# mitenjain/nanopore

Hardware: AMD Instinct MI355X
Metric: DP cells/sec (banded pair-HMM realign: forward + backward + posterior per cell) (higher is better)
Workload: dtype f32

## Files before the change

### nanopore_amd/csrc/npr_api_internal.h

```cpp
#pragma once
#include <hip/hip_runtime.h>

#include <algorithm>
#include <atomic>
#include <chrono>
#include <cmath>
#include <cstdio>
#include <cstdlib>
#include <cstring>
#include <exception>
#include <memory>
#include <mutex>
#include <new>
#include <numeric>
#include <string>
#include <thread>
#include <type_traits>
#include <vector>

#include "npr_device.h"
#include "npr_internal.h"
#include "npr_sched.h"
#include "npr_threads.h"

using namespace npr;

struct npr_plan {
    Plan plan;
};

namespace npr_impl {
struct MeaScratch;

struct DeviceArena {
    static constexpr size_t kPad = 1024;
    std::mutex mu;
    char *F = nullptr;
    std::atomic<size_t> cells{0};
    std::atomic<uint64_t> epoch{1};
    int users = 0;
};
constexpr int kMaxDevices = 64;
extern DeviceArena g_arena[kMaxDevices];
}
using namespace npr_impl;

struct npr_ctx {
    int device = -1;
    hipStream_t stream = nullptr;
    hipEvent_t ev0 = nullptr, ev1 = nullptr;
    static constexpr int kSideStreams = 6;
    hipStream_t side[kSideStreams] = {};
    hipEvent_t side_done[kSideStreams] = {};
    int cu_count = 0;
    size_t total_mem = 0;
    bool model_set[NPR_MAX_MODELS] = {};
    DevModel models[NPR_MAX_MODELS];
    DevModel *d_models = nullptr;
    std::string last_error;
    int host_threads = 1;
    DeviceArena *arena = nullptr;
    int overlap = 0;
    int64_t opt[NPR_OPT_COUNT] = {};
    static constexpr size_t kArenaPad = DeviceArena::kPad;
    float *arena_Fx = nullptr;
    size_t arena_fx_cells = 0;
    void *pin_pairs = nullptr;
    size_t pin_pairs_bytes = 0;
    std::vector<hipEvent_t> ops_events;
    struct HostWords {
        std::unique_ptr<uint32_t[]> p;
        int64_t cap = 0;
    };
    std::vector<HostWords> packed_pool;
    void take_packed(int64_t words, std::unique_ptr<uint32_t[]> &p, int64_t &cap) {
        for (size_t i = 0; i < packed_pool.size(); ++i)
            if (packed_pool[i].cap >= words) {
                p = std::move(packed_pool[i].p), cap = packed_pool[i].cap;
                packed_pool.erase(packed_pool.begin() + static_cast<std::ptrdiff_t>(i));
                return;
            }
    }
    void give_packed(std::unique_ptr<uint32_t[]> &p, int64_t cap) {
        if (!p) return;
        if (packed_pool.size() < 2) {
            packed_pool.push_back(HostWords{std::move(p), cap});
            return;
        }
        auto &smallest = *std::min_element(packed_pool.begin(), packed_pool.end(), [](const HostWords &x, const HostWords &y) { return x.cap < y.cap; });
        if (smallest.cap < cap) smallest.p = std::move(p), smallest.cap = cap;
    }
    void *pin_stage = nullptr;
    size_t pin_stage_bytes = 0;
    MeaScratch *mea = nullptr;
    struct Cached {
        void *p;
        size_t bytes;
    };
    std::vector<Cached> cache;
    size_t cache_bytes = 0;
    void cache_flush() {
        for (const Cached &c : cache) (void)hipFree(c.p);
        cache.clear();
        cache_bytes = 0;
// ... 113 lines not shown
struct StageTimer {
    bool on;
    std::chrono::steady_clock::time_point t0;
    const char *what;
    explicit StageTimer(const char *w) : on(std::getenv("NPR_TIMING") != nullptr), t0(std::chrono::steady_clock::now()), what(w) {}
    void lap(const char *label) {
        if (!on) return;
        const auto t1 = std::chrono::steady_clock::now();
        std::fprintf(stderr, "[npr timing] %s / %s: %.1f ms\n", what, label, std::chrono::duration<double, std::milli>(t1 - t0).count());
        t0 = t1;
    }
};

}
using namespace npr_impl;

struct npr_batch {
    npr_ctx *ctx = nullptr;
    npr_params params{};
    int64_t n_reads = 0;
    std::vector<int64_t> ref_len, read_len;
    std::vector<int64_t> gstart;
    std::vector<int32_t> ref_id;
    std::vector<int32_t> guide_ops;
    std::vector<int64_t> guide_off;
    std::vector<int32_t> read_status;
    std::vector<int32_t> read_first_task, read_ntasks;
    std::vector<Task> tasks;
    std::vector<int32_t> task_of;
    std::vector<int64_t> task_cells;
    std::vector<TaskOut> outs;
    std::vector<uint8_t> task_rerun;
    npr_batch_stats stats{};
    DevBuf<Task> d_tasks;
    DevBuf<TaskOut> d_outs;
    DevBuf<int32_t> d_queue;
    DevBuf<uint8_t> d_seq;
    DevBuf<int32_t> d_lo, d_n;
    DevBuf<uint32_t> d_coff;
    DevBuf<uint32_t> d_ctl;
    DevBuf<Stripe> d_stripes;
    DevBuf<uint32_t> d_rowmask;
    DevBuf<PlanSeg> d_pseg;
    DevBuf<int64_t> d_region;
    std::vector<int64_t> region_end;
    size_t scratch_cells = 0;
    bool variable_regions = false;
    bool pair_rs = false;
    DevBuf<int32_t> d_px, d_py;
    DevBuf<float> d_pp;
    int64_t slot_stride = 0;
    struct Launch {
        int cls;
        int first, count, grid, wcap;
        int threads;
        size_t lds;
        int64_t cells;
        int64_t width;
        int slot_base;
        int region_first;
        bool own_regions;
    };
    std::vector<Launch> launches;
    DevBuf<float> d_ring;
    bool ran = false, finished = false;
    int32_t finish_stage = 0;
    std::vector<npr_read_result> results;
    std::vector<int64_t> ops_off;
    std::unique_ptr<int32_t[]> ops;
    int64_t ops_words = 0, ops_cap = 0;
    std::unique_ptr<uint32_t[]> packed;
    int64_t packed_cap = 0;
    bool have_pairs_form = false, have_packed_form = false;
    bool ops_from_guide = false;
    bool rs_staged = false;
    int rs_shift = 0;
    std::vector<int64_t> rs_columns, rs_kept;
    DevBuf<int32_t> d_rs_gy;
    DevBuf<int64_t> d_rs_gx_off;
    std::vector<int64_t> pair_off;
    std::vector<Pair> pairs;
    bool pairs_ready = false;
    std::vector<int64_t> task_dst;
    const uint32_t *dev_ops = nullptr;
    const int64_t *dev_od = nullptr;
    uint64_t dev_ops_epoch = 0;
    std::unique_ptr<char[]> text;
    int64_t text_cap = 0;
    std::vector<int64_t> text_off;
    bool text_ready = false, words_on_device = false;
};

struct npr_pileup {
    npr_ctx *ctx = nullptr;
    std::vector<int64_t> len;
    std::vector<int64_t> base;
    int64_t rows = 0;
    DevBuf<int32_t> tab;
    DevBuf<int32_t> diff;
    DevBuf<int32_t> tile;
    DevBuf<int64_t> dbase;
    DevBuf<int32_t> bad;
};

namespace npr_impl {

inline bool build_stair_schedule(const Segment &s, int R, int NW, uint32_t *ctl, int64_t *cells) {
    if (s.n.empty()) return false;
    return stair_schedule(s.lo.data(), s.n.data(), s.D(), s.max_width, R, NW, ctl, cells);
}

}
using namespace npr_impl;

namespace npr_impl {
enum { K_STAIR = 0, K_WIDE = 1, K_GENERIC_LDS = 2, K_GENERIC_GLOBAL = 3, K_TILE = 4, K_MID = 5, K_RS = 6, K_TILE_RS = 7 };
struct KClass {
    int kind, R, NW;
    int slots() const { return 64 * R * NW; }
};
constexpr int kClasses = 19;
constexpr KClass kClassTab[kClasses] = {{K_STAIR, 1, 1}, {K_STAIR, 2, 1}, {K_STAIR, 4, 1}, {K_WIDE, 2, 4}, {K_WIDE, 2, 8},
                                        {K_WIDE, 4, 8}, {K_WIDE, 4, 12}, {K_GENERIC_LDS, 0, 0}, {K_GENERIC_LDS, 0, 0},
                                        {K_GENERIC_LDS, 0, 0}, {K_GENERIC_GLOBAL, 0, 0}, {K_TILE, 2, 0},
                                        {K_MID, 1, 1}, {K_MID, 2, 1}, {K_MID, 4, 1},
                                        {K_RS, 1, 1}, {K_RS, 2, 1}, {K_RS, 4, 1},
                                        {K_TILE_RS, 2, 0}};
constexpr int kFirstGeneric = 7, kTileClass = 11, kFirstPair = 12, kFirstRs = 15, kTileRsClass = 18, kQueueSlots = 24;
inline bool is_register_class(int c) { return kClassTab[c].kind <= K_WIDE || kClassTab[c].kind == K_MID || kClassTab[c].kind == K_RS; }
inline bool is_one_wave_kind(int kind) { return kind == K_STAIR || kind == K_RS; }
inline bool is_tile_kind(int kind) { return kind == K_TILE || kind == K_TILE_RS; }
inline int stair_waves_per_cu(int R) { return R == 1 ? 28 : (R == 2 ? 24 : 12); }
inline int rs_waves_per_cu(int R) { return R == 1 ? 28 : (R == 2 ? 28 : 16); }

inline bool rs_model_ok(const DevModel &m) {
    double grow = 0.0, em_max = 0.0;
    for (int x = 0; x < 4; ++x)
        for (int y = 0; y < 4; ++y) em_max = std::max(em_max, static_cast<double>(m.em[x * 5 + y]));
    for (int to = 0; to < 5; ++to) {
        double col = 0.0, e = em_max;
        for (int from = 0; from < 5; ++from) col += static_cast<double>(m.T[from * 5 + to]);
        if (to > 0) {
            e = 0.0;
            for (int b2 = 0; b2 < 5; ++b2) e = std::max(e, static_cast<double>((to == 1 || to == 3) ? m.ex[to * 5 + b2] : m.ey[to * 5 + b2]));
        }
        grow = std::max(grow, col * e);
    }
    auto emax = [&](int st) {
        if (st == 0) return em_max;
        double e = 0.0;
        for (int b2 = 0; b2 < 5; ++b2) e = std::max(e, static_cast<double>((st == 1 || st == 3) ? m.ex[st * 5 + b2] : m.ey[st * 5 + b2]));
        return e;
    };
    for (int from = 0; from < 5; ++from) {
        double row = 0.0;
        for (int to = 0; to < 5; ++to) row += static_cast<double>(m.T[from * 5 + to]) * emax(to);
        grow = std::max(grow, row);
    }
    return grow <= std::exp2(6.0 / NPR_RS_K);
}

struct ModelShape { bool sw, flat_gaps, flat, rs_ok; };
inline ModelShape model_shape(const npr_ctx *ctx) {
    ModelShape s{false, true, false, true};
    for (int sl = 0; sl < NPR_MAX_MODELS; ++sl) {
        if (!ctx->model_set[sl]) continue;
        const DevModel &m = ctx->models[sl];
        if (m.T[1 * 5 + 2] != 0.f || m.T[2 * 5 + 1] != 0.f) s.sw = true;
        if (!rs_model_ok(m)) s.rs_ok = false;
        for (int b2 = 0; b2 < 5; ++b2)
            if (m.ex[5 + b2] != 0.25f || m.ex[15 + b2] != 0.25f || m.ey[10 + b2] != 0.25f || m.ey[20 + b2] != 0.25f) s.flat_gaps = false;
    }
    s.flat = !s.sw && s.flat_gaps;
    return s;
}

inline void build_stripes(const Segment &s, int R, Stripe *out, int64_t *rows_out) {
    const int64_t S = (s.xe - s.xs) / (64 * R) + 1;
    int64_t rows;
    if (out) {
        rows = stripe_ranges(s.lo.data(), s.n.data(), s.D(), s.xe - s.xs, R, &out[1].df, &out[1].dl, static_cast<int>(sizeof(Stripe) / sizeof(int32_t)));
        stripe_fill(out, s.xe - s.xs, R);
    } else {
        thread_local std::vector<int32_t> df, dl;
        df.resize(S), dl.resize(S);
        rows = stripe_ranges(s.lo.data(), s.n.data(), s.D(), s.xe - s.xs, R, df.data(), dl.data(), 1);
    }
    if (rows_out) *rows_out = rows;
}
inline int64_t stripes_of(const Segment &s, int R) { return (s.xe - s.xs) / (64 * R) + 1; }
}
using namespace npr_impl;

namespace npr_impl {
int32_t rescore_stage(npr_batch *b);
KernelArgs make_args(npr_batch *b);
int32_t ensure_coff(npr_batch *b);
int32_t release_scratch(npr_ctx *ctx, bool caches_only);
void ensure_packed_form(npr_batch *b);
int32_t grow_pin_stage(npr_ctx *ctx, size_t bytes, const char *what);
int32_t device_words_text(npr_batch *b, const int64_t *d_off, const uint32_t *d_words, char *lend, size_t lend_bytes);
using PieceMove = void (*)(void *dst, const void *pin, int64_t lo, int64_t hi);
struct PiecedFetch {
    const void *dev;
    void *dst;
    int64_t count;
    size_t elem;
    int64_t per_piece, round_to;
    PieceMove move;
    const char *what_pin, *what_d2h;
};
int32_t fetch_pieced(npr_ctx *ctx, const PiecedFetch &f);
int32_t fetch_device_words(npr_batch *b);
}
```

### nanopore_amd/csrc/npr_finish.cpp

```cpp
#include "npr_api_internal.h"

namespace npr_impl {

static int32_t grow_pinned(npr_ctx *ctx, void *&p, size_t &have, size_t bytes, const char *what) {
    if (bytes <= have) return NPR_OK;
    if (p) (void)hipHostFree(p);
    p = nullptr, have = 0;
    const hipError_t e = hipHostMalloc(&p, bytes + bytes / 4, hipHostMallocDefault);
    if (e != hipSuccess) return fail(ctx, NPR_ERR_NOMEM, what, e);
    have = bytes + bytes / 4;
    return NPR_OK;
}
int32_t grow_pin_pairs(npr_ctx *ctx, size_t bytes, const char *what) { return grow_pinned(ctx, ctx->pin_pairs, ctx->pin_pairs_bytes, bytes, what); }
int32_t grow_pin_stage(npr_ctx *ctx, size_t bytes, const char *what) { return grow_pinned(ctx, ctx->pin_stage, ctx->pin_stage_bytes, bytes, what); }

int32_t fetch_pieced(npr_ctx *ctx, const PiecedFetch &f) {
    if (f.count <= 0) return NPR_OK;
    const int32_t grown = grow_pin_pairs(ctx, f.elem * static_cast<size_t>(f.count), f.what_pin);
    if (grown != NPR_OK) return grown;
    constexpr int64_t kMaxPieces = 48;
    const int64_t pieces = std::min(kMaxPieces, (f.count + f.per_piece - 1) / f.per_piece);
    const int64_t piece = ((f.count + pieces - 1) / pieces + f.round_to - 1) / f.round_to * f.round_to;
    while (static_cast<int64_t>(ctx->ops_events.size()) < pieces) {
        hipEvent_t ev;
// ... 112 lines not shown
        int64_t runs = 0, cols = 0, kept = 0;
        for (int64_t q = b->guide_off[i]; q < b->guide_off[i + 1]; ++q) {
            const int32_t len = b->guide_ops[2 * q + 1];
            kept += len > 0;
            if (b->guide_ops[2 * q] == NPR_OP_M && len > 0) ++runs, cols += len;
        }
        b->rs_columns[i] = cols, b->rs_kept[i] = kept, run_off[i + 1] = b->read_status[i] == NPR_OK ? runs : 0;
    });
    if (ctx->opt[NPR_OPT_HOST_MEA] != 0 || n == 0) return NPR_OK;
    int e2 = 0;
    (void)std::frexp(b->params.posterior_threshold, &e2);
    const int shift = 24 - e2;
    if (!(b->params.posterior_threshold > 0.0) || shift > 44 || shift < 0) return NPR_OK;
    for (int64_t i = 0; i < n; ++i) {
        if (b->rs_columns[i] >= (int64_t(1) << (53 - shift))) return NPR_OK;
        run_off[i + 1] += run_off[i];
        gx_off[i + 1] = gx_off[i] + (b->read_status[i] == NPR_OK ? b->ref_len[i] + 1 : 0);
    }
    std::vector<int32_t> runs_v;
    int32_t *runs = nullptr;
    const size_t run_bytes = sizeof(int32_t) * 3 * static_cast<size_t>(run_off[n]);
    if (ctx->pin_stage && ctx->pin_stage_bytes >= run_bytes) runs = static_cast<int32_t *>(ctx->pin_stage);
    else runs_v.resize(3 * static_cast<size_t>(run_off[n])), runs = runs_v.data();
    parallel_for(n, ctx->host_threads, [&](int64_t i) {
        if (b->read_status[i] != NPR_OK) return;
        int32_t *out = runs + 3 * run_off[i];
        int64_t x = 0, y = 0;
        for (int64_t q = b->guide_off[i]; q < b->guide_off[i + 1]; ++q) {
            const int32_t op = b->guide_ops[2 * q], len = b->guide_ops[2 * q + 1];
            if (op == NPR_OP_M) {
                if (len > 0) out[0] = static_cast<int32_t>(x), out[1] = static_cast<int32_t>(y), out[2] = len, out += 3;
                x += len, y += len;
            } else if (op == NPR_OP_I) {
                y += len;
            } else {
                x += len;
            }
        }
    });
    tm.lap("runs");
    DevBuf<int64_t> d_run_off;
    DevBuf<int32_t> d_runs;
    hipError_t e;
    if ((e = d_run_off.alloc_from(ctx, n + 1)) != hipSuccess || (e = b->d_rs_gx_off.alloc_from(ctx, n + 1)) != hipSuccess ||
        (e = d_runs.alloc_from(ctx, std::max<size_t>(3 * static_cast<size_t>(run_off[n]), 1))) != hipSuccess ||
        (e = b->d_rs_gy.alloc_from(ctx, std::max<int64_t>(gx_off[n], 1))) != hipSuccess)
        return fail(ctx, NPR_ERR_NOMEM, "npr_batch_create: hipMalloc (rescore tables)", e);
    HIP_TRY(ctx, hipMemcpyAsync(d_run_off.p, run_off.data(), sizeof(int64_t) * (n + 1), hipMemcpyHostToDevice, ctx->stream));
    HIP_TRY(ctx, hipMemcpyAsync(b->d_rs_gx_off.p, gx_off.data(), sizeof(int64_t) * (n + 1), hipMemcpyHostToDevice, ctx->stream));
    if (run_bytes) HIP_TRY(ctx, hipMemcpyAsync(d_runs.p, runs, run_bytes, hipMemcpyHostToDevice, ctx->stream));
    HIP_TRY(ctx, hipMemsetAsync(b->d_rs_gy.p, 0xff, sizeof(int32_t) * std::max<int64_t>(gx_off[n], 1), ctx->stream));
    RescoreArgs ra{static_cast<int32_t>(n), 0, d_run_off.p, d_runs.p, b->d_rs_gx_off.p, b->d_rs_gy.p, nullptr, nullptr, nullptr, nullptr, nullptr, nullptr, shift};
    const int rc = launch_rescore_table(ra, ctx->stream);
    if (rc != 0) return fail(ctx, NPR_ERR_HIP, "k_rescore_table launch", static_cast<hipError_t>(rc));
    HIP_TRY(ctx, hipStreamSynchronize(ctx->stream));
    tm.lap("table");
    b->rs_shift = shift, b->rs_staged = true;
    return NPR_OK;
}

int32_t rescore_sum(npr_batch *b, std::vector<double> &score) {
    npr_ctx *ctx = b->ctx;
    const int64_t n = b->n_reads, ntasks = static_cast<int64_t>(b->tasks.size());
    DevBuf<unsigned long long> d_sum;
    hipError_t e;
    if ((e = d_sum.alloc_from(ctx, n)) != hipSuccess) return fail(ctx, NPR_ERR_NOMEM, "npr_batch_finish: hipMalloc (rescore sums)", e);
    HIP_TRY(ctx, hipMemsetAsync(d_sum.p, 0, sizeof(unsigned long long) * n, ctx->stream));
    RescoreArgs ra{static_cast<int32_t>(n), static_cast<int32_t>(ntasks), nullptr, nullptr, b->d_rs_gx_off.p, b->d_rs_gy.p, b->d_tasks.p, b->d_outs.p,
                   b->d_px.p, b->d_py.p, b->d_pp.p, d_sum.p, b->rs_shift};
    const int rc = launch_rescore_sum(ra, ctx->stream);
    if (rc != 0) return fail(ctx, NPR_ERR_HIP, "k_rescore_sum launch", static_cast<hipError_t>(rc));
    std::vector<unsigned long long> sum(n);
    HIP_TRY(ctx, hipMemcpyAsync(sum.data(), d_sum.p, sizeof(unsigned long long) * n, hipMemcpyDeviceToHost, ctx->stream));
    HIP_TRY(ctx, hipStreamSynchronize(ctx->stream));
    score.assign(n, 0.0);
    for (int64_t i = 0; i < n; ++i)
        if (b->rs_columns[i] > 0) score[i] = std::ldexp(static_cast<double>(sum[i]), -b->rs_shift) / static_cast<double>(b->rs_columns[i]);
    return NPR_OK;
}


constexpr int32_t kHostStage = 1;

struct MeaPlan {
    int64_t n = 0, total = 0, n_pieces = 0;
    size_t ntask_map = 0, n_cnt = 1;
    int64_t span = 0;
    bool sort_in_lds = true;
    std::vector<int64_t> offs;
    int64_t stride() const { return n + 1; }
    int64_t *arr(int k) { return offs.data() + k * stride(); }
    int64_t cols() const { return offs[2 * stride() - 1]; }
    int64_t ops_bound() const { return offs[4 * stride() - 1]; }
    std::vector<int32_t> order;
    std::vector<int32_t> pieces_head;
};

constexpr int64_t kOffArrays = 5, kSortedArrays = 8, kSmallArrays = 6, kVrecWords = 4;

MeaPlan plan_mea(const npr_batch *b) {
    MeaPlan p;
    const int64_t n = p.n = b->n_reads;
    p.offs.assign(kOffArrays * p.stride(), 0);
    int64_t *const rx = p.arr(0), *const ry = p.arr(1), *const rp = p.arr(2), *const ot = p.arr(3), *const cnt_off = p.arr(4);
    for (int64_t i = 0; i < n; ++i) {
        const bool ok = b->results[i].status == NPR_OK;
        const int64_t lX = ok ? b->ref_len[i] : 0, lY = ok ? b->read_len[i] : 0, np = ok ? b->pair_off[i + 1] - b->pair_off[i] : 0;
        rx[i + 1] = rx[i] + lX + 1;
        ry[i + 1] = ry[i] + lY;
        rp[i + 1] = rp[i] + np;
        ot[i + 1] = ot[i] + 3 * std::min({np, lX, lY}) + 2;
    }
    p.total = rp[n];
    const int64_t lds_span = b->ctx->opt[NPR_OPT_MEA_GLOBAL_SORT] != 0 ? 0 : kMeaSortLdsSpan;
    int64_t cnt_total = 0;
    for (int64_t i = 0; i < n; ++i) {
        const int64_t sp = std::max(rx[i + 1] - rx[i], ry[i + 1] - ry[i]);
        cnt_off[i] = -1;
        if (sp <= lds_span) p.span = std::max(p.span, (rx[i + 1] - rx[i]) + (ry[i + 1] - ry[i]));
        else cnt_off[i] = cnt_total, cnt_total += rx[i + 1] - rx[i];
    }
    cnt_off[n] = -1;
    p.sort_in_lds = cnt_total == 0;
    p.n_cnt = p.sort_in_lds ? 1 : static_cast<size_t>(cnt_total);
    p.ntask_map = b->task_of.size();
    p.order.resize(n);
    std::iota(p.order.begin(), p.order.end(), 0);
    std::stable_sort(p.order.begin(), p.order.end(), [&](int32_t x, int32_t y) { return rp[x + 1] - rp[x] > rp[y + 1] - rp[y]; });
    constexpr int64_t kMaxPieces = 64, kLanesWanted = 64 * 5 * 256;
    const int64_t kPiecePairs = std::min<int64_t>(2048, std::max<int64_t>(128, p.total / kLanesWanted));
    std::vector<int32_t> np(n);
    for (int64_t i = 0; i < n; ++i) np[i] = static_cast<int32_t>(std::min(kMaxPieces, std::max<int64_t>(1, (rp[i + 1] - rp[i] + kPiecePairs - 1) / kPiecePairs))), p.n_pieces += np[i];
    p.pieces_head.resize(3 * n + 2 * p.n_pieces);
    int32_t *const t_np = p.pieces_head.data(), *const t_poff = t_np + n, *const t_pboff = t_poff + n, *const t_lr = t_pboff + n, *const t_lp = t_lr + p.n_pieces;
    int64_t at = 0;
    for (int64_t k = 0; k < n; ++k) {
        const int32_t r = p.order[k];
        t_np[r] = np[r], t_poff[r] = static_cast<int32_t>(at), t_pboff[r] = static_cast<int32_t>(at + k);
        for (int32_t j = 0; j < np[r]; ++j) t_lr[at + j] = r, t_lp[at + j] = j;
        at += np[r];
    }
    return p;
}

static_assert(kSortedArrays % kVrecWords == 0, "vrec starts on a 16-byte boundary of m.sorted (the arena's tables start 256-byte aligned)");
inline int64_t sorted_stride(const MeaPlan &p) { return p.total + 1; }

template <typename F>
hipError_t for_each_table(MeaScratch &m, const MeaPlan &p, F &&f) {
    hipError_t e = hipSuccess;
    auto one = [&](auto &buf, int64_t count) {
        if (e == hipSuccess) e = f(buf, static_cast<size_t>(count));
    };
    one(m.off, kOffArrays * p.stride());
    one(m.mass, p.n);
    one(m.od, p.n + 1);
    one(m.cnt, p.n_cnt);
    one(m.start, p.n_cnt);
    one(m.col, p.cols() + 1);
    one(m.sorted, kSortedArrays * sorted_stride(p) + kVrecWords * (p.total + 2) + sorted_stride(p));
    one(m.small, kSmallArrays * p.n);
    one(m.tmp, 2 * p.ops_bound());
    one(m.map, 3 * p.n + p.ntask_map);
    one(m.dense, p.ops_bound());
    one(m.pieces, 4 * p.n_pieces + 4 * p.n);
    return e;
}

inline size_t table_align(size_t bytes) { return (bytes + 255) & ~size_t(255); }

int32_t carve_tables(npr_ctx *ctx, MeaScratch &m, const MeaPlan &p, size_t need) {
    if (poison_byte() >= 0) {
        HIP_TRY(ctx, hipStreamSynchronize(ctx->stream));
        poison(ctx->arena->F, need);
    }
    char *cur = ctx->arena->F;
    (void)for_each_table(m, p, [&](auto &buf, size_t count) {
        using T = std::remove_pointer_t<decltype(buf.p)>;
        buf.borrow(reinterpret_cast<T *>(cur), count);
        cur += table_align(sizeof(T) * count);
        return hipSuccess;
    });
    return NPR_OK;
}

int32_t obtain_tables(npr_ctx *ctx, MeaScratch &m, const MeaPlan &p, std::unique_lock<std::mutex> &arena_lock) {
    size_t need = 0;
    (void)for_each_table(m, p, [&](auto &buf, size_t count) { return need += table_align(sizeof(*buf.p) * count), hipSuccess; });
    auto arena_fits = [&] { return ctx->arena->F && need <= static_cast<size_t>(ctx->arena->cells.load()) * 8; };
    const bool fits = arena_fits();
    if (!ctx->overlap && fits) return carve_tables(ctx, m, p, need);
    if (for_each_table(m, p, [](auto &buf, size_t count) { return buf.reserve(count); }) == hipSuccess) return NPR_OK;
    (void)hipGetLastError();
    if (!(ctx->overlap && fits)) return kHostStage;
    (void)for_each_table(m, p, [](auto &buf, size_t) { return buf.release(), hipSuccess; });
    ctx->cache_flush();
    arena_lock.lock();
    if (!arena_fits()) return kHostStage;
    ++ctx->arena->epoch;
    return carve_tables(ctx, m, p, need);
}

int32_t upload_tables(npr_batch *b, const MeaPlan &p, MeaScratch &m, MeaArgs &a) {
    npr_ctx *ctx = b->ctx;
    const int64_t n = p.n, P = p.n_pieces, so = p.stride(), ss = sorted_stride(p);
    a.tasks = b->d_tasks.p, a.outs = b->d_outs.p, a.ntasks = static_cast<int32_t>(b->tasks.size()), a.n_reads = static_cast<int32_t>(n);
    a.px = b->d_px.p, a.py = b->d_py.p, a.pp = b->d_pp.p;
    a.rx_off = m.off.p, a.ry_off = m.off.p + so, a.rp_off = m.off.p + 2 * so, a.ot_off = m.off.p + 3 * so, a.cnt_off = m.off.p + 4 * so;
    a.cnt = m.cnt.p, a.start = m.start.p, a.colsum = m.col.p;
    a.sx = m.sorted.p, a.sy = m.sorted.p + ss, a.sq = m.sorted.p + 2 * ss, a.back = m.sorted.p + 3 * ss;
    a.kx = m.sorted.p + 4 * ss, a.ky = m.sorted.p + 5 * ss, a.kq = m.sorted.p + 6 * ss, a.kback = m.sorted.p + 7 * ss;
    a.vrec = reinterpret_cast<int4 *>(m.sorted.p + kSortedArrays * ss);
    a.sw = m.sorted.p + kSortedArrays * ss + kVrecWords * (p.total + 2);
    a.best_who = m.small.p, a.read_flag = m.small.p + n, a.n_ops = m.small.p + 2 * n, a.chain_len = m.small.p + 3 * n, a.kept = m.small.p + 4 * n, a.max_run = m.small.p + 5 * n;
    a.chain_mass = m.mass.p;
    int32_t *const read_first = m.map.p, *const read_ntasks = read_first + n, *const task_of = read_ntasks + n, *const order = task_of + p.ntask_map;
    a.read_first = read_first, a.read_ntasks = read_ntasks, a.task_of = task_of, a.order = order;
    int32_t *const lanes = m.pieces.p + 3 * n;
    a.np = m.pieces.p, a.poff = m.pieces.p + n, a.pboff = m.pieces.p + 2 * n, a.lane_read = lanes, a.lane_piece = lanes + P, a.pbest = lanes + 2 * P, a.pb = lanes + 3 * P;
    a.n_pieces = static_cast<int32_t>(P);
    a.ops_tmp = m.tmp.p, a.od_off = m.od.p;
    a.gap_gamma = b->params.gap_gamma, a.match_gamma = b->params.match_gamma;
    a.ring = 8192;
    a.ring_only = ctx->opt[NPR_OPT_MEA_RING_ONLY] != 0 ? 1 : 0;
    a.sort_lds_bytes = static_cast<int32_t>(4 * p.span);
    a.sort_threads = ctx->overlap == 1 ? 512 : 0;
    a.any_global_sort = p.sort_in_lds ? 0 : 1;
    HIP_TRY(ctx, hipMemcpyAsync(read_first, b->read_first_task.data(), sizeof(int32_t) * n, hipMemcpyHostToDevice, ctx->stream));
    HIP_TRY(ctx, hipMemcpyAsync(read_ntasks, b->read_ntasks.data(), sizeof(int32_t) * n, hipMemcpyHostToDevice, ctx->stream));
    HIP_TRY(ctx, hipMemcpyAsync(task_of, b->task_of.data(), sizeof(int32_t) * p.ntask_map, hipMemcpyHostToDevice, ctx->stream));
    HIP_TRY(ctx, hipMemcpyAsync(order, p.order.data(), sizeof(int32_t) * n, hipMemcpyHostToDevice, ctx->stream));
    HIP_TRY(ctx, hipMemcpyAsync(m.pieces.p, p.pieces_head.data(), sizeof(int32_t) * p.pieces_head.size(), hipMemcpyHostToDevice, ctx->stream));
    HIP_TRY(ctx, hipMemcpyAsync(m.off.p, p.offs.data(), m.off.bytes(), hipMemcpyHostToDevice, ctx->stream));
    HIP_TRY(ctx, hipMemsetAsync(m.small.p, 0, m.small.bytes(), ctx->stream));
    return NPR_OK;
}

int32_t run_chain(npr_ctx *ctx, const MeaArgs &a, MeaScratch &m, std::vector<int32_t> &small, std::vector<int64_t> &mass) {
    int rc = launch_mea_sort(a, ctx->stream);
    if (rc == 0) rc = launch_mea_chain(a, ctx->stream);
    if (rc != 0) return fail(ctx, NPR_ERR_HIP, "MEA kernel launch", static_cast<hipError_t>(rc));
    small.resize(m.small.count), mass.resize(m.mass.count);
    HIP_TRY(ctx, hipMemcpyAsync(small.data(), m.small.p, m.small.bytes(), hipMemcpyDeviceToHost, ctx->stream));
    HIP_TRY(ctx, hipMemcpyAsync(mass.data(), m.mass.p, m.mass.bytes(), hipMemcpyDeviceToHost, ctx->stream));
    HIP_TRY(ctx, hipStreamSynchronize(ctx->stream));
    return NPR_OK;
}

int32_t collect_results(npr_batch *b, const std::vector<int32_t> &small, const std::vector<int64_t> &mass, int32_t &longest) {
    const int64_t n = b->n_reads;
    const int32_t *flag = small.data() + n, *nops = small.data() + 2 * n, *clen = small.data() + 3 * n, *max_run = small.data() + 5 * n;
    for (int64_t i = 0; i < n; ++i)
        if (b->results[i].status == NPR_OK && flag[i] == NPR_ERR_CAPACITY) return kHostStage;
    std::vector<int64_t> &od = b->ops_off;
    od.assign(n + 1, 0);
    longest = 0;
    for (int64_t i = 0; i < n; ++i) {
        npr_read_result &r = b->results[i];
        if (r.status == NPR_OK && flag[i] != 0) r.status = flag[i];
        const int64_t k = r.status == NPR_OK ? nops[i] : 0;
        od[i + 1] = od[i] + k;
        if (k) longest = std::max(longest, max_run[i]);
        r.n_ops = k;
        r.score = (r.status == NPR_OK && clen[i] > 0) ? static_cast<double>(mass[i]) / (static_cast<double>(clen[i]) * PROB_ONE) : 0.0;
    }
    b->ops_words = 2 * od[n];
    return NPR_OK;
}

int32_t gather_ops(npr_batch *b, MeaScratch &m, MeaArgs &a, uint16_t *dense16) {
    npr_ctx *ctx = b->ctx;
    HIP_TRY(ctx, hipMemcpyAsync(m.od.p, b->ops_off.data(), m.od.bytes(), hipMemcpyHostToDevice, ctx->stream));
    if (b->ops_off[b->n_reads] == 0) return NPR_OK;
    a.ops_dense = m.dense.p, a.ops_dense16 = dense16;
    const int rc = launch_mea_gather(a, ctx->stream);
    return rc == 0 ? NPR_OK : fail(ctx, NPR_ERR_HIP, "k_mea_gather launch", static_cast<hipError_t>(rc));
}
void words_stay_on_device(npr_batch *b, const MeaScratch &m) { b->dev_ops = m.dense.p, b->dev_od = m.od.p, b->dev_ops_epoch = b->ctx->arena->epoch; }

int32_t hand_over_words(npr_batch *b, MeaScratch &m, MeaArgs &a, int32_t longest) {
    npr_ctx *ctx = b->ctx;
    const int64_t words = b->ops_off[b->n_reads];
    b->have_pairs_form = false, b->have_packed_form = true;
    if (words > b->packed_cap) ctx->take_packed(words, b->packed, b->packed_cap);
    if (words > b->packed_cap) {
        b->packed.reset(new uint32_t[words + words / 8]);
        b->packed_cap = words + words / 8;
    }
    if (words == 0) return NPR_OK;
    const bool narrow = longest < (1 << 14) && ctx->opt[NPR_OPT_MEA_WIDE_OPS] == 0 &&
                        sizeof(uint16_t) * static_cast<size_t>(words) <= m.sorted.bytes();
    int32_t rc = gather_ops(b, m, a, narrow ? reinterpret_cast<uint16_t *>(m.sorted.p) : nullptr);
    if (rc != NPR_OK) return rc;
    PiecedFetch f{m.dense.p, b->packed.get(), words, sizeof(uint32_t), int64_t(1) << 20, 64, nullptr, "npr_batch_finish: hipHostMalloc", "npr_batch_finish: D2H of the ops"};
    f.move = [](void *dst, const void *pin, int64_t lo, int64_t hi) {
        std::memcpy(static_cast<uint32_t *>(dst) + lo, static_cast<const uint32_t *>(pin) + lo, sizeof(uint32_t) * static_cast<size_t>(hi - lo));
    };
    if (narrow) {
        f.dev = a.ops_dense16, f.elem = sizeof(uint16_t);
        f.move = [](void *dst, const void *pin, int64_t lo, int64_t hi) {
            uint32_t *out = static_cast<uint32_t *>(dst);
            const uint16_t *src = static_cast<const uint16_t *>(pin);
            for (int64_t i = lo; i < hi; ++i) out[i] = src[i];
        };
    }
    if ((rc = fetch_pieced(ctx, f)) != NPR_OK) return rc;
    words_stay_on_device(b, m);
    return NPR_OK;
}

int32_t hand_over_text(npr_batch *b, MeaScratch &m, MeaArgs &a) {
    b->have_pairs_form = false, b->have_packed_form = false, b->words_on_device = true;
    int32_t rc = gather_ops(b, m, a, nullptr);
    if (rc == NPR_OK) rc = device_words_text(b, m.od.p, m.dense.p, reinterpret_cast<char *>(m.sorted.p), m.sorted.bytes());
    if (rc == NPR_OK) words_stay_on_device(b, m);
    return rc;
}

int32_t device_mea(npr_batch *b) {
    npr_ctx *ctx = b->ctx;
    std::unique_lock<std::mutex> arena_lock(ctx->arena->mu, std::defer_lock);
    if (!ctx->overlap) arena_lock.lock();
    ++ctx->arena->epoch;
    StageTimer tm("device_mea");
    const MeaPlan p = plan_mea(b);
    if (!ctx->mea) ctx->mea = new MeaScratch;
    MeaScratch &m = *ctx->mea;
    MeaArgs a{};
    std::vector<int32_t> small;
    std::vector<int64_t> mass;
    int32_t longest = 0;
    int32_t rc = obtain_tables(ctx, m, p, arena_lock);
    if (rc == NPR_OK) rc = upload_tables(b, p, m, a);
    if (rc == NPR_OK) rc = run_chain(ctx, a, m, small, mass);
    if (rc != NPR_OK) return rc;
    tm.lap("sort + chain + trace");
    if ((rc = collect_results(b, small, mass, longest)) != NPR_OK) return rc;
    rc = ctx->opt[NPR_OPT_FINISH_TEXT] != 0 ? hand_over_text(b, m, a) : hand_over_words(b, m, a, longest);
    if (rc == NPR_OK) tm.lap("gather + D2H of the ops");
    return rc;
}


int32_t task_results(npr_batch *b) {
    npr_ctx *ctx = b->ctx;
    const int64_t ntasks = static_cast<int64_t>(b->tasks.size());
    const int64_t n = b->n_reads;
    std::vector<int64_t> &dst = b->task_dst;
    dst.assign(ntasks + 1, 0);
    if (ntasks) HIP_TRY(ctx, hipMemcpy(b->outs.data(), b->d_outs.p, b->d_outs.bytes(), hipMemcpyDeviceToHost));
    for (int64_t k = 0; k < ntasks; ++k) dst[k + 1] = dst[k] + std::min(b->outs[k].npairs, b->tasks[k].pair_cap);
    b->results.assign(n, npr_read_result{});
    b->pair_off.assign(n + 1, 0);
    b->pairs_ready = false;
    b->text_ready = false, b->words_on_device = false;
    const double LN2 = 0.69314718055994530942;
    for (int64_t i = 0; i < n; ++i) {
        npr_read_result &r = b->results[i];
        r.status = b->read_status[i];
        r.n_segments = b->read_ntasks[i];
        int64_t c = 0;
        if (r.status == NPR_OK)
            for (int32_t s = 0; s < b->read_ntasks[i]; ++s) {
                const int32_t k = b->task_of[b->read_first_task[i] + s];
                const TaskOut &o = b->outs[k];
                if (o.status != NPR_OK && r.status == NPR_OK) r.status = o.status;
                r.cells += b->task_cells[k];
                if (o.tot_m > 0.f) r.loglik += (std::log2(static_cast<double>(o.tot_m)) + o.tot_e) * LN2;
                if (o.btot_m > 0.f) r.loglik_bwd += (std::log2(static_cast<double>(o.btot_m)) + o.btot_e) * LN2;
                c += dst[k + 1] - dst[k];
            }
        r.n_pairs = c;
        b->pair_off[i + 1] = b->pair_off[i] + c;
    }
    return NPR_OK;
}

int32_t gated_device_mea(npr_batch *b) {
    npr_ctx *ctx = b->ctx;
    int64_t scratch = 0;
    for (int64_t i = 0; i < b->n_reads; ++i) scratch += 8 * (b->ref_len[i] + 1) + 4 * b->read_len[i] + 36 * std::min(b->ref_len[i], b->read_len[i]) + 128;
    scratch += 48 * b->pair_off[b->n_reads];
    size_t mem_free = 0, mem_total = 0;
    const size_t arena_bytes = ctx->arena->cells.load() * 8;
    if (static_cast<size_t>(scratch) <= arena_bytes ||
        (hipMemGetInfo(&mem_free, &mem_total) == hipSuccess && static_cast<size_t>(scratch) < mem_free / 2))
        return device_mea(b);
    return kHostStage;
}

void host_rescore(npr_batch *b, const std::vector<double> *dev_score) {
    const int64_t n = b->n_reads;
    b->ops_off.assign(n + 1, 0);
    parallel_for(n, b->ctx->host_threads, [&](int64_t i) {
        npr_read_result &r = b->results[i];
        if (r.status != NPR_OK) return;
        r.n_ops = b->rs_kept[i], b->ops_off[i + 1] = b->rs_kept[i];
        r.score = dev_score ? (*dev_score)[i]
                            : rescore(b->guide_ops.data() + 2 * b->guide_off[i], b->guide_off[i + 1] - b->guide_off[i], b->pairs.data() + b->pair_off[i], r.n_pairs);
    });
    for (int64_t i = 0; i < n; ++i) b->ops_off[i + 1] += b->ops_off[i];
    b->ops_words = 2 * b->ops_off[n];
    b->ops_from_guide = true, b->have_pairs_form = false, b->have_packed_form = false;
}

void host_mea(npr_batch *b, StageTimer &tm) {
    const int64_t n = b->n_reads;
    std::vector<std::vector<int32_t>> per_read_ops(n);
    parallel_for(n, b->ctx->host_threads, [&](int64_t i) {
        npr_read_result &r = b->results[i];
        if (r.status != NPR_OK) return;
        const int32_t rc = mea_cigar(b->ref_len[i], b->read_len[i], b->pairs.data() + b->pair_off[i], r.n_pairs, b->params.gap_gamma, b->params.match_gamma, per_read_ops[i], r.score);
        if (rc != NPR_OK) r.status = rc;
        r.n_ops = static_cast<int64_t>(per_read_ops[i].size() / 2);
    });
    tm.lap("MEA + cigar");
    b->ops_off.assign(n + 1, 0);
    for (int64_t i = 0; i < n; ++i) b->ops_off[i + 1] = b->ops_off[i] + static_cast<int64_t>(per_read_ops[i].size() / 2);
    b->ops_words = 2 * b->ops_off[n];
    if (b->ops_words > b->ops_cap) {
// ... 216 lines not shown
```

### nanopore_amd/csrc/npr_mea.hip

```cpp
#include <hip/hip_runtime.h>

#include "npr_device.h"

namespace npr {
namespace {

constexpr int64_t P1 = PROB_ONE;
constexpr int WAVE = 64;
constexpr int SORT_THREADS = 1024;

__device__ __forceinline__ int rdlane(int v, int j) { return __builtin_amdgcn_readlane(v, j); }
__device__ __forceinline__ int64_t rdlane64(int64_t v, int j) {
    const int lo = __builtin_amdgcn_readlane(static_cast<int>(v), j);
    const int hi = __builtin_amdgcn_readlane(static_cast<int>(v >> 32), j);
    return (static_cast<int64_t>(hi) << 32) | static_cast<uint32_t>(lo);
}
__device__ __forceinline__ void wave_sync() {
    __builtin_amdgcn_fence(__ATOMIC_RELEASE, "wavefront");
    __builtin_amdgcn_wave_barrier();
    __builtin_amdgcn_fence(__ATOMIC_ACQUIRE, "wavefront");
}
__device__ __forceinline__ bool beats(int64_t s, int w, int64_t os, int ow) { return s > os || (s == os && w > ow); }

__device__ __forceinline__ int mea_task_pairs(const TaskOut &o, const Task &tk) { return o.status == NPR_OK ? min(max(o.npairs, 0), tk.pair_cap) : 0; }
// ... 636 lines not shown
    while (piece-- > 0) {
    int i = !alive ? -1 : __builtin_amdgcn_readfirstlane(by_id ? pbest[piece] : a.best_who[r]);
    while (i >= 0) {
        const int cb = max(i - (WAVE - 1), 0), idx = min(cb + lane, i);
        const int vb = back[idx], vx = sx[idx], vy = sy[idx], vq = sq[idx];
        const int rel = (vb - cb) & (WAVE - 1);
        const bool diag = vb >= cb && __shfl(vx, rel) == vx - 1 && __shfl(vy, rel) == vy - 1;
        int nxt = diag ? rel : lane, val = diag ? vq : 0;
#pragma unroll
        for (int k = 0; k < 6; ++k) {
            val += __shfl(val, nxt);
            nxt = __shfl(nxt, nxt);
        }
        while (i >= cb) {
            const int l = i - cb, h = rdlane(nxt, l);
            const int x = rdlane(vx, l), y = rdlane(vy, l), hx = rdlane(vx, h), hy = rdlane(vy, h);
            emit(NPR_OP_I, cy - y - 1);
            emit(NPR_OP_D, cx - x - 1);
            emit(NPR_OP_M, x - hx + 1);
            cx = hx, cy = hy, mass += rdlane(val, l) + rdlane(vq, h), len += x - hx + 1;
            const int to = rdlane(vb, h);
            if (to >= i) {
                broken = true;
                i = -1;
                break;
            }
            i = to;
        }
    }
    if (broken) break;
    }
    emit(NPR_OP_I, cy);
    emit(NPR_OP_D, cx);
    if (hop >= 0 && p > lo) {
        --p;
        if (lane == 0) *p = make_int2(hop, hlen);
        longest = max(longest, hlen);
    }
    if (lane == 0) {
        if (broken) a.read_flag[r] = NPR_ERR_INVALID;
        a.max_run[r] = longest;
        a.n_ops[r] = broken ? 0 : static_cast<int>(reinterpret_cast<int2 *>(a.ops_tmp) + a.ot_off[r + 1] - p);
        a.chain_len[r] = len;
        a.chain_mass[r] = mass;
    }
}

__global__ void __launch_bounds__(256) k_mea_gather(MeaArgs a) {
    for (int r = blockIdx.x; r < a.n_reads; r += gridDim.x) {
        const int n = static_cast<int>(a.od_off[r + 1] - a.od_off[r]);
        const int2 *src = reinterpret_cast<const int2 *>(a.ops_tmp) + a.ot_off[r + 1] - a.n_ops[r];
        uint32_t *dst = a.ops_dense + a.od_off[r];
        uint16_t *const dst16 = a.ops_dense16 ? a.ops_dense16 + a.od_off[r] : nullptr;
        for (int i = threadIdx.x; i < n; i += blockDim.x) {
            const uint32_t w = static_cast<uint32_t>(src[i].y) << 2 | static_cast<uint32_t>(src[i].x);
            dst[i] = w;
            if (dst16) dst16[i] = static_cast<uint16_t>(w);
        }
    }
}

}

size_t mea_chain_lds_bytes(int ring) { return static_cast<size_t>(ring) * 12 + WAVE * (8 + 4 + 4); }

int launch_mea_sort(const MeaArgs &a, void *stream) {
    hipStream_t s = static_cast<hipStream_t>(stream);
    if (a.sort_lds_bytes > 0) {
        const hipError_t e = hipFuncSetAttribute(reinterpret_cast<const void *>(k_mea_sort_lds), hipFuncAttributeMaxDynamicSharedMemorySize, a.sort_lds_bytes);
        if (e != hipSuccess) return static_cast<int>(e);
        hipLaunchKernelGGL(k_mea_sort_lds, dim3(a.n_reads), dim3(a.sort_threads >= WAVE && a.sort_threads < SORT_THREADS ? a.sort_threads & ~(WAVE - 1) : SORT_THREADS), a.sort_lds_bytes, s, a);
    }
    if (a.any_global_sort) {
        const int tg = a.ntasks < 8192 ? (a.ntasks > 0 ? a.ntasks : 1) : 8192;
        hipLaunchKernelGGL(k_mea_zero, dim3(a.n_reads), dim3(256), 0, s, a);
        hipLaunchKernelGGL(k_mea_count, dim3(tg), dim3(256), 0, s, a);
        hipLaunchKernelGGL(k_mea_scan, dim3(a.n_reads), dim3(256), 0, s, a);
        hipLaunchKernelGGL(k_mea_scatter, dim3(tg), dim3(256), 0, s, a);
        hipLaunchKernelGGL(k_mea_weight_sorted, dim3(a.n_reads), dim3(256), 0, s, a);
    }
    return static_cast<int>(hipGetLastError());
}

int launch_mea_chain(const MeaArgs &a, void *stream) {
    hipStream_t s = static_cast<hipStream_t>(stream);
    const size_t lds = mea_chain_lds_bytes(a.ring);
    const hipError_t e = hipFuncSetAttribute(reinterpret_cast<const void *>(k_mea_chain), hipFuncAttributeMaxDynamicSharedMemorySize, static_cast<int>(lds));
    if (e != hipSuccess) return static_cast<int>(e);
    const int lanes_lds = LWIN * WAVE * static_cast<int>(sizeof(int64_t));
    const hipError_t e2 = hipFuncSetAttribute(reinterpret_cast<const void *>(k_mea_chain_lanes), hipFuncAttributeMaxDynamicSharedMemorySize, lanes_lds);
    if (e2 != hipSuccess) return static_cast<int>(e2);
    hipLaunchKernelGGL(k_mea_weigh, dim3(a.n_reads), dim3(WAVE), 0, s, a);
    hipLaunchKernelGGL(k_mea_cuts, dim3(a.n_reads), dim3(WAVE), 0, s, a);
    hipLaunchKernelGGL(k_mea_chain_lanes, dim3((a.n_pieces + WAVE - 1) / WAVE), dim3(WAVE), lanes_lds, s, a);
    hipLaunchKernelGGL(k_mea_chain, dim3(a.n_reads < 512 ? (a.n_reads > 0 ? a.n_reads : 1) : 512), dim3(WAVE), lds, s, a);
    hipLaunchKernelGGL(k_mea_trace, dim3(a.n_reads), dim3(WAVE), 0, s, a);
    return static_cast<int>(hipGetLastError());
}

int launch_mea_gather(const MeaArgs &a, void *stream) {
    const int g = a.n_reads < 8192 ? a.n_reads : 8192;
    hipLaunchKernelGGL(k_mea_gather, dim3(g), dim3(256), 0, static_cast<hipStream_t>(stream), a);
    return static_cast<int>(hipGetLastError());
}

}
```

Measured before the change: 383.4 billion.

## Restructure MEA host planning: pinned staging, radix order, cached static plan, overlapped piece upload

Host-side MEA planning now writes its offsets, task maps, order and piece tables directly into a pinned buffer, so several small pageable uploads become two larger copies. The stable_sort by pair count becomes an LSD radix sort. Per-read offsets that depend only on lengths and status are cached across calls on the batch. The weigh kernel is launched separately so the piece table can be built on the host while sort and weigh run on the GPU. This targets host planning and upload latency around the MEA stage, at the cost of more complex buffer aliasing and a cache that assumes ref and read lengths do not change while status is unchanged.

After: 386.3 billion (median of 6 runs). About the same (+0.8%).

```diff
diff --git a/nanopore_amd/csrc/npr_api_internal.h b/nanopore_amd/csrc/npr_api_internal.h
--- a/nanopore_amd/csrc/npr_api_internal.h
+++ b/nanopore_amd/csrc/npr_api_internal.h
@@ -20,6 +20,7 @@
 
 #include "npr_device.h"
 #include "npr_internal.h"
+#include "npr_mea_plan.h"
 #include "npr_sched.h"
 #include "npr_threads.h"
 
@@ -299,6 +300,7 @@
     std::vector<Pair> pairs;
     bool pairs_ready = false;
     std::vector<int64_t> task_dst;
+    MeaStaticPlan mea_static;
     const uint32_t *dev_ops = nullptr;
     const int64_t *dev_od = nullptr;
     uint64_t dev_ops_epoch = 0;
@@ -409,6 +411,9 @@
 }
 using namespace npr_impl;
 
+namespace npr {
+int launch_mea_weigh(const MeaArgs &a, void *stream);
+}
 namespace npr_impl {
 int32_t rescore_stage(npr_batch *b);
 KernelArgs make_args(npr_batch *b);
diff --git a/nanopore_amd/csrc/npr_finish.cpp b/nanopore_amd/csrc/npr_finish.cpp
--- a/nanopore_amd/csrc/npr_finish.cpp
+++ b/nanopore_amd/csrc/npr_finish.cpp
@@ -218,65 +218,39 @@
 
 constexpr int32_t kHostStage = 1;
 
-struct MeaPlan {
-    int64_t n = 0, total = 0, n_pieces = 0;
-    size_t ntask_map = 0, n_cnt = 1;
-    int64_t span = 0;
-    bool sort_in_lds = true;
-    std::vector<int64_t> offs;
-    int64_t stride() const { return n + 1; }
-    int64_t *arr(int k) { return offs.data() + k * stride(); }
-    int64_t cols() const { return offs[2 * stride() - 1]; }
-    int64_t ops_bound() const { return offs[4 * stride() - 1]; }
-    std::vector<int32_t> order;
-    std::vector<int32_t> pieces_head;
-};
-
-constexpr int64_t kOffArrays = 5, kSortedArrays = 8, kSmallArrays = 6, kVrecWords = 4;
-
-MeaPlan plan_mea(const npr_batch *b) {
-    MeaPlan p;
+
+constexpr int64_t kSortedArrays = 8, kSmallArrays = 6, kVrecWords = 4;
+
+int32_t stage_plan(npr_batch *b, MeaPlan &p) {
+    npr_ctx *ctx = b->ctx;
     const int64_t n = p.n = b->n_reads;
-    p.offs.assign(kOffArrays * p.stride(), 0);
-    int64_t *const rx = p.arr(0), *const ry = p.arr(1), *const rp = p.arr(2), *const ot = p.arr(3), *const cnt_off = p.arr(4);
-    for (int64_t i = 0; i < n; ++i) {
-        const bool ok = b->results[i].status == NPR_OK;
-        const int64_t lX = ok ? b->ref_len[i] : 0, lY = ok ? b->read_len[i] : 0, np = ok ? b->pair_off[i + 1] - b->pair_off[i] : 0;
-        rx[i + 1] = rx[i] + lX + 1;
-        ry[i + 1] = ry[i] + lY;
-        rp[i + 1] = rp[i] + np;
-        ot[i + 1] = ot[i] + 3 * std::min({np, lX, lY}) + 2;
-    }
-    p.total = rp[n];
+    p.ntask_map = b->task_of.size();
+    const size_t off_words = static_cast<size_t>(kOffArrays * p.stride()), map_words = static_cast<size_t>(3 * n) + p.ntask_map;
+    const size_t piece_words = static_cast<size_t>(3 * n + 2 * mea_pieces_bound(n, b->pair_off[n]));
+    const int32_t grown = grow_pin_pairs(ctx, sizeof(int64_t) * off_words + sizeof(int32_t) * (map_words + piece_words + static_cast<size_t>(n)), "npr_batch_finish: hipHostMalloc");
+    if (grown != NPR_OK) return grown;
+    p.offs = static_cast<int64_t *>(ctx->pin_pairs);
+    int32_t *const map = reinterpret_cast<int32_t *>(p.offs + off_words);
+    std::copy(b->read_first_task.begin(), b->read_first_task.end(), map);
+    std::copy(b->read_ntasks.begin(), b->read_ntasks.end(), map + n);
+    std::copy(b->task_of.begin(), b->task_of.end(), map + 2 * n);
+    p.order = map + 2 * n + p.ntask_map;
+    p.pieces_head = map + map_words;
+    return NPR_OK;
+}
+
+void plan_head(npr_batch *b, MeaPlan &p) {
+    const int64_t n = p.n;
     const int64_t lds_span = b->ctx->opt[NPR_OPT_MEA_GLOBAL_SORT] != 0 ? 0 : kMeaSortLdsSpan;
-    int64_t cnt_total = 0;
-    for (int64_t i = 0; i < n; ++i) {
-        const int64_t sp = std::max(rx[i + 1] - rx[i], ry[i + 1] - ry[i]);
-        cnt_off[i] = -1;
-        if (sp <= lds_span) p.span = std::max(p.span, (rx[i + 1] - rx[i]) + (ry[i + 1] - ry[i]));
-        else cnt_off[i] = cnt_total, cnt_total += rx[i + 1] - rx[i];
-    }
-    cnt_off[n] = -1;
-    p.sort_in_lds = cnt_total == 0;
-    p.n_cnt = p.sort_in_lds ? 1 : static_cast<size_t>(cnt_total);
-    p.ntask_map = b->task_of.size();
-    p.order.resize(n);
-    std::iota(p.order.begin(), p.order.end(), 0);
-    std::stable_sort(p.order.begin(), p.order.end(), [&](int32_t x, int32_t y) { return rp[x + 1] - rp[x] > rp[y + 1] - rp[y]; });
-    constexpr int64_t kMaxPieces = 64, kLanesWanted = 64 * 5 * 256;
-    const int64_t kPiecePairs = std::min<int64_t>(2048, std::max<int64_t>(128, p.total / kLanesWanted));
-    std::vector<int32_t> np(n);
-    for (int64_t i = 0; i < n; ++i) np[i] = static_cast<int32_t>(std::min(kMaxPieces, std::max<int64_t>(1, (rp[i + 1] - rp[i] + kPiecePairs - 1) / kPiecePairs))), p.n_pieces += np[i];
-    p.pieces_head.resize(3 * n + 2 * p.n_pieces);
-    int32_t *const t_np = p.pieces_head.data(), *const t_poff = t_np + n, *const t_pboff = t_poff + n, *const t_lr = t_pboff + n, *const t_lp = t_lr + p.n_pieces;
-    int64_t at = 0;
-    for (int64_t k = 0; k < n; ++k) {
-        const int32_t r = p.order[k];
-        t_np[r] = np[r], t_poff[r] = static_cast<int32_t>(at), t_pboff[r] = static_cast<int32_t>(at + k);
-        for (int32_t j = 0; j < np[r]; ++j) t_lr[at + j] = r, t_lp[at + j] = j;
-        at += np[r];
-    }
-    return p;
+    MeaStaticPlan &s = b->mea_static;
+    bool same = s.lds_span == lds_span && static_cast<int64_t>(s.status.size()) == n;
+    for (int64_t i = 0; same && i < n; ++i) same = s.status[i] == b->results[i].status;
+    if (!same) {
+        std::vector<int32_t> status(n);
+        for (int64_t i = 0; i < n; ++i) status[i] = b->results[i].status;
+        mea_plan_static(n, status.data(), b->ref_len.data(), b->read_len.data(), lds_span, s);
+    }
+    mea_plan_head(p, s, b->ref_len.data(), b->read_len.data(), b->pair_off.data(), p.pieces_head + 3 * n + 2 * mea_pieces_bound(n, b->pair_off[n]));
 }
 
 static_assert(kSortedArrays % kVrecWords == 0, "vrec starts on a 16-byte boundary of m.sorted (the arena's tables start 256-byte aligned)");
@@ -362,20 +336,28 @@
     a.sort_lds_bytes = static_cast<int32_t>(4 * p.span);
     a.sort_threads = ctx->overlap == 1 ? 512 : 0;
     a.any_global_sort = p.sort_in_lds ? 0 : 1;
-    HIP_TRY(ctx, hipMemcpyAsync(read_first, b->read_first_task.data(), sizeof(int32_t) * n, hipMemcpyHostToDevice, ctx->stream));
-    HIP_TRY(ctx, hipMemcpyAsync(read_ntasks, b->read_ntasks.data(), sizeof(int32_t) * n, hipMemcpyHostToDevice, ctx->stream));
-    HIP_TRY(ctx, hipMemcpyAsync(task_of, b->task_of.data(), sizeof(int32_t) * p.ntask_map, hipMemcpyHostToDevice, ctx->stream));
-    HIP_TRY(ctx, hipMemcpyAsync(order, p.order.data(), sizeof(int32_t) * n, hipMemcpyHostToDevice, ctx->stream));
-    HIP_TRY(ctx, hipMemcpyAsync(m.pieces.p, p.pieces_head.data(), sizeof(int32_t) * p.pieces_head.size(), hipMemcpyHostToDevice, ctx->stream));
-    HIP_TRY(ctx, hipMemcpyAsync(m.off.p, p.offs.data(), m.off.bytes(), hipMemcpyHostToDevice, ctx->stream));
+    HIP_TRY(ctx, hipMemcpyAsync(m.off.p, p.offs, m.off.bytes(), hipMemcpyHostToDevice, ctx->stream));
+    HIP_TRY(ctx, hipMemcpyAsync(m.map.p, p.order - 2 * n - p.ntask_map, m.map.bytes(), hipMemcpyHostToDevice, ctx->stream));
     HIP_TRY(ctx, hipMemsetAsync(m.small.p, 0, m.small.bytes(), ctx->stream));
     return NPR_OK;
 }
 
-int32_t run_chain(npr_ctx *ctx, const MeaArgs &a, MeaScratch &m, std::vector<int32_t> &small, std::vector<int64_t> &mass) {
+int32_t run_chain(npr_ctx *ctx, MeaPlan &p, const MeaArgs &a, MeaScratch &m, std::vector<int32_t> &small, std::vector<int64_t> &mass, StageTimer &tm) {
+    const bool pieces_first = ctx->overlap != 0;
+    auto pieces_up = [&]() -> int32_t {
+        mea_plan_pieces(p);
+        HIP_TRY(ctx, hipMemcpyAsync(m.pieces.p, p.pieces_head, sizeof(int32_t) * p.pieces_head_count(), hipMemcpyHostToDevice, ctx->stream));
+        return NPR_OK;
+    };
+    int32_t up = pieces_first ? pieces_up() : NPR_OK;
+    if (up != NPR_OK) return up;
     int rc = launch_mea_sort(a, ctx->stream);
-    if (rc == 0) rc = launch_mea_chain(a, ctx->stream);
+    if (rc == 0) rc = launch_mea_weigh(a, ctx->stream);
     if (rc != 0) return fail(ctx, NPR_ERR_HIP, "MEA kernel launch", static_cast<hipError_t>(rc));
+    tm.lap("tables, upload, sort + weigh launched");
+    if (!pieces_first && (up = pieces_up()) != NPR_OK) return up;
+    if ((rc = launch_mea_chain(a, ctx->stream)) != 0) return fail(ctx, NPR_ERR_HIP, "MEA kernel launch", static_cast<hipError_t>(rc));
+    tm.lap("pieces planned + up, chain launched");
     small.resize(m.small.count), mass.resize(m.mass.count);
     HIP_TRY(ctx, hipMemcpyAsync(small.data(), m.small.p, m.small.bytes(), hipMemcpyDeviceToHost, ctx->stream));
     HIP_TRY(ctx, hipMemcpyAsync(mass.data(), m.mass.p, m.mass.bytes(), hipMemcpyDeviceToHost, ctx->stream));
@@ -459,19 +441,24 @@
     if (!ctx->overlap) arena_lock.lock();
     ++ctx->arena->epoch;
     StageTimer tm("device_mea");
-    const MeaPlan p = plan_mea(b);
+    MeaPlan p;
+    int32_t rc = stage_plan(b, p);
+    if (rc != NPR_OK) return rc;
+    plan_head(b, p);
+    tm.lap("plan: offsets and order");
     if (!ctx->mea) ctx->mea = new MeaScratch;
     MeaScratch &m = *ctx->mea;
     MeaArgs a{};
     std::vector<int32_t> small;
     std::vector<int64_t> mass;
     int32_t longest = 0;
-    int32_t rc = obtain_tables(ctx, m, p, arena_lock);
+    rc = obtain_tables(ctx, m, p, arena_lock);
     if (rc == NPR_OK) rc = upload_tables(b, p, m, a);
-    if (rc == NPR_OK) rc = run_chain(ctx, a, m, small, mass);
+    if (rc == NPR_OK) rc = run_chain(ctx, p, a, m, small, mass, tm);
     if (rc != NPR_OK) return rc;
-    tm.lap("sort + chain + trace");
+    tm.lap("the kernels (waited for)");
     if ((rc = collect_results(b, small, mass, longest)) != NPR_OK) return rc;
+    tm.lap("results collected");
     rc = ctx->opt[NPR_OPT_FINISH_TEXT] != 0 ? hand_over_text(b, m, a) : hand_over_words(b, m, a, longest);
     if (rc == NPR_OK) tm.lap("gather + D2H of the ops");
     return rc;
diff --git a/nanopore_amd/csrc/npr_mea.hip b/nanopore_amd/csrc/npr_mea.hip
--- a/nanopore_amd/csrc/npr_mea.hip
+++ b/nanopore_amd/csrc/npr_mea.hip
@@ -742,6 +742,11 @@
     return static_cast<int>(hipGetLastError());
 }
 
+int launch_mea_weigh(const MeaArgs &a, void *stream) {
+    hipLaunchKernelGGL(k_mea_weigh, dim3(a.n_reads), dim3(WAVE), 0, static_cast<hipStream_t>(stream), a);
+    return static_cast<int>(hipGetLastError());
+}
+
 int launch_mea_chain(const MeaArgs &a, void *stream) {
     hipStream_t s = static_cast<hipStream_t>(stream);
     const size_t lds = mea_chain_lds_bytes(a.ring);
@@ -750,7 +755,6 @@
     const int lanes_lds = LWIN * WAVE * static_cast<int>(sizeof(int64_t));
     const hipError_t e2 = hipFuncSetAttribute(reinterpret_cast<const void *>(k_mea_chain_lanes), hipFuncAttributeMaxDynamicSharedMemorySize, lanes_lds);
     if (e2 != hipSuccess) return static_cast<int>(e2);
-    hipLaunchKernelGGL(k_mea_weigh, dim3(a.n_reads), dim3(WAVE), 0, s, a);
     hipLaunchKernelGGL(k_mea_cuts, dim3(a.n_reads), dim3(WAVE), 0, s, a);
     hipLaunchKernelGGL(k_mea_chain_lanes, dim3((a.n_pieces + WAVE - 1) / WAVE), dim3(WAVE), lanes_lds, s, a);
     hipLaunchKernelGGL(k_mea_chain, dim3(a.n_reads < 512 ? (a.n_reads > 0 ? a.n_reads : 1) : 512), dim3(WAVE), lds, s, a);
diff --git a/nanopore_amd/csrc/npr_mea_plan.h b/nanopore_amd/csrc/npr_mea_plan.h
--- /dev/null
+++ b/nanopore_amd/csrc/npr_mea_plan.h
@@ -0,0 +1,115 @@
+#pragma once
+#include <algorithm>
+#include <cstdint>
+#include <vector>
+
+#include "nprealign.h"
+
+namespace npr_impl {
+
+constexpr int64_t kOffArrays = 5;
+
+struct MeaPlan {
+    int64_t n = 0, total = 0, n_pieces = 0;
+    size_t ntask_map = 0, n_cnt = 1;
+    int64_t span = 0;
+    bool sort_in_lds = true;
+    int64_t *offs = nullptr;
+    int64_t stride() const { return n + 1; }
+    int64_t *arr(int k) const { return offs + k * stride(); }
+    int64_t cols() const { return offs[2 * stride() - 1]; }
+    int64_t ops_bound() const { return offs[4 * stride() - 1]; }
+    int32_t *order = nullptr;
+    int32_t *pieces_head = nullptr;
+    size_t pieces_head_count() const { return static_cast<size_t>(3 * n + 2 * n_pieces); }
+};
+
+struct MeaStaticPlan {
+    std::vector<int32_t> status;
+    int64_t lds_span = -1;
+    std::vector<int64_t> offs;
+    int64_t span = 0, cnt_total = 0;
+};
+
+inline void mea_plan_static(int64_t n, const int32_t *status, const int64_t *ref_len, const int64_t *read_len, int64_t lds_span, MeaStaticPlan &s) {
+    s.status.assign(status, status + n), s.lds_span = lds_span;
+    s.offs.assign(3 * (n + 1), 0);
+    int64_t *const rx = s.offs.data(), *const ry = rx + n + 1, *const cnt_off = ry + n + 1;
+    s.span = 0, s.cnt_total = 0;
+    for (int64_t i = 0; i < n; ++i) {
+        const bool ok = status[i] == NPR_OK;
+        const int64_t nx = (ok ? ref_len[i] : 0) + 1, ny = ok ? read_len[i] : 0;
+        rx[i + 1] = rx[i] + nx, ry[i + 1] = ry[i] + ny;
+        cnt_off[i] = -1;
+        if (std::max(nx, ny) <= lds_span) s.span = std::max(s.span, nx + ny);
+        else cnt_off[i] = s.cnt_total, s.cnt_total += nx;
+    }
+    cnt_off[n] = -1;
+}
+
+inline void mea_order_desc(const int64_t *key, int64_t n, int32_t *order, int32_t *tmp) {
+    constexpr int kBits = 11;
+    int64_t top = 0;
+    for (int64_t i = 0; i < n; ++i) top = std::max(top, key[i]);
+    for (int64_t i = 0; i < n; ++i) order[i] = static_cast<int32_t>(i);
+    int32_t *from = order, *to = tmp;
+    for (int shift = 0; shift < 64 && (top >> shift) != 0; shift += kBits) {
+        int64_t first[(1 << kBits) + 1] = {};
+        for (int64_t i = 0; i < n; ++i) ++first[(((top - key[i]) >> shift) & ((1 << kBits) - 1)) + 1];
+        for (int d = 0; d < (1 << kBits); ++d) first[d + 1] += first[d];
+        for (int64_t i = 0; i < n; ++i) to[first[((top - key[from[i]]) >> shift) & ((1 << kBits) - 1)]++] = from[i];
+        std::swap(from, to);
+    }
+    if (from != order) std::copy(from, from + n, order);
+}
+
+inline int64_t mea_piece_pairs(int64_t total) {
+    constexpr int64_t kLanesWanted = 64 * 5 * 256;
+    return std::min<int64_t>(2048, std::max<int64_t>(128, total / kLanesWanted));
+}
+constexpr int64_t kMeaMaxPieces = 64;
+inline int64_t mea_pieces_bound(int64_t n, int64_t pairs) { return n + pairs / 128; }
+
+inline void mea_plan_head(MeaPlan &p, const MeaStaticPlan &s, const int64_t *ref_len, const int64_t *read_len, const int64_t *pair_off, int32_t *scratch) {
+    const int64_t n = p.n;
+    int64_t *const rx = p.arr(0), *const rp = p.arr(2), *const ot = p.arr(3), *const cnt_off = p.arr(4);
+    std::copy(s.offs.begin(), s.offs.begin() + 2 * (n + 1), rx);
+    std::copy(s.offs.begin() + 2 * (n + 1), s.offs.end(), cnt_off);
+    rp[0] = 0, ot[0] = 0;
+    for (int64_t i = 0; i < n; ++i) {
+        const bool ok = s.status[i] == NPR_OK;
+        const int64_t lX = ok ? ref_len[i] : 0, lY = ok ? read_len[i] : 0, np = ok ? pair_off[i + 1] - pair_off[i] : 0;
+        rp[i + 1] = rp[i] + np;
+        ot[i + 1] = ot[i] + 3 * std::min({np, lX, lY}) + 2;
+    }
+    p.total = rp[n];
+    p.span = s.span;
+    p.sort_in_lds = s.cnt_total == 0;
+    p.n_cnt = p.sort_in_lds ? 1 : static_cast<size_t>(s.cnt_total);
+    int32_t *const t_np = p.pieces_head;
+    {
+        std::vector<int64_t> count(n);
+        for (int64_t i = 0; i < n; ++i) count[i] = rp[i + 1] - rp[i];
+        mea_order_desc(count.data(), n, p.order, scratch);
+        const int64_t piece_pairs = mea_piece_pairs(p.total);
+        p.n_pieces = 0;
+        for (int64_t i = 0; i < n; ++i) {
+            t_np[i] = static_cast<int32_t>(std::min(kMeaMaxPieces, std::max<int64_t>(1, (count[i] + piece_pairs - 1) / piece_pairs)));
+            p.n_pieces += t_np[i];
+        }
+    }
+}
+
+inline void mea_plan_pieces(MeaPlan &p) {
+    const int64_t n = p.n;
+    int32_t *const t_np = p.pieces_head, *const t_poff = t_np + n, *const t_pboff = t_poff + n, *const t_lr = t_pboff + n, *const t_lp = t_lr + p.n_pieces;
+    int64_t at = 0;
+    for (int64_t k = 0; k < n; ++k) {
+        const int32_t r = p.order[k];
+        t_poff[r] = static_cast<int32_t>(at), t_pboff[r] = static_cast<int32_t>(at + k);
+        for (int32_t j = 0; j < t_np[r]; ++j) t_lr[at + j] = r, t_lp[at + j] = j;
+        at += t_np[r];
+    }
+}
+
+}
```
